# gaebor/w-fsa

Hardware: AMD Instinct MI355X
Metric: forward-backward strings/sec @1/2/4/8 GPU; log-lik rel-err vs MKL ref (higher is better)
Workload: dtype f64

## Files before the change

include/wfsa_dev.h:

```cpp
#ifndef WFSA_DEV_H
#define WFSA_DEV_H

#include <stdint.h>

#ifdef __cplusplus
extern "C" {
#endif

#define WFSA_OK 0
#define WFSA_ERR_ARG (-1)
#define WFSA_ERR_HIP (-2)
#define WFSA_ERR_MODEL (-3)
#define WFSA_ERR_CAPACITY (-4)
#define WFSA_ERR_RCCL (-5)
#define WFSA_ERR_NODEV (-6)

typedef struct wfsa_dev wfsa_dev;

typedef struct {
    int32_t n_states;
    int32_t start;
    int32_t end;
    int32_t n_params;
    const int32_t* em_ptr;
// ... 19 lines not shown
    int64_t stream_bytes;
    int64_t bubble_words;
    int64_t n_bubbles;
    int64_t fb_launches;
    double fb_kernel_ms;
    double last_fb_kernel_ms;
    double last_compiled_ms;
    double last_call_ms;
    int64_t last_live_edges;
    int32_t tier1_strings;
    int32_t waves_per_block;
    double prepare_ms;
    double compiled_kernel_ms;
    int32_t graph;
    int32_t dense;
    int64_t host_steps;
    double host_begin_ms, host_overlap_ms, host_wait_ms, host_post_ms;
    int32_t dense_rows, dense_steps, dense_np;
    int32_t tier2_strings;
    int32_t wave_strings;
    int64_t wave_row_entries;
    int64_t wave_pair_edges;
    int32_t comm_ranks;
    int32_t comm_peer;
    int64_t slot_chunks;
    int32_t max_group_chunks;
    int32_t wave_pull;
    int32_t dense_blas;
    int32_t qn_inkernel_waves;
    int32_t qn_batches;
    int32_t stream_block;
    int32_t stream_w_lds;
    int32_t stream_wide;
    int32_t stream_multi;
    int32_t stream_delta;
    int32_t bubbles_fused;
    int32_t grad_tables;
    int32_t wave_lgrad;
    int64_t ll_dot_launches;
    double best_path_ms;
    double kbest_path_ms;
    double sample_path_ms;
    double posterior_count_ms;
    double byte_marginal_ms;
    int64_t shaped_bubbles;
    int64_t mixed_shape_waves;
    int64_t small_bubbles_a;
    int64_t small_bubbles_b;
    int64_t big_bubbles;
    int32_t max_bubble_nodes;
    int32_t max_bubble_edges;
    double generate_ms;
    double dense_bp_tables_ms, dense_bp_forward_ms, dense_bp_backtrack_ms;
} wfsa_dev_stats;

int wfsa_dev_create(int device, wfsa_dev** out);
void wfsa_dev_destroy(wfsa_dev* ctx);
const char* wfsa_dev_last_error(void);

int wfsa_dev_load_model(wfsa_dev* ctx, const wfsa_model_desc* model);
int wfsa_dev_load_corpus(wfsa_dev* ctx, const uint8_t* sym, const int64_t* off,
                         const double* p, int64_t n_strings);

int wfsa_dev_recognize(wfsa_dev* ctx, uint8_t* recognized, double* path_count,
                       uint8_t* used_param);

int wfsa_dev_sym_factor(wfsa_dev* ctx, int64_t n, const double* a, int64_t inertia[3], double* log_abs_det,
                        int32_t* det_sign);
int wfsa_dev_sym_solve(wfsa_dev* ctx, double* b);
int wfsa_dev_sym_factor_coo(wfsa_dev* ctx, int64_t n, int64_t nnz, const int32_t* i, const int32_t* j,
                            const double* v, double* b, int64_t inertia[3], double* log_abs_det, int32_t* det_sign,
                            int32_t* method);

int wfsa_dev_load_paths(wfsa_dev* ctx, int32_t n_params, int64_t n_paths, const int64_t* prow, const int32_t* pcol,
                        const double* pdata, int64_t n_strings, const int64_t* mrow, const int64_t* mcol,
                        const double* p);

int wfsa_dev_rmin(wfsa_dev* ctx, double* rmin, int64_t* string_index);

int wfsa_dev_best_paths(wfsa_dev* ctx, const double* w_full, double* best_logw, int64_t* n_entries);
int wfsa_dev_best_paths_get(wfsa_dev* ctx, int64_t* prow, int32_t* pidx);

int wfsa_dev_dense_best_paths(wfsa_dev* ctx, const double* w_full, double* best_logw ,
                              int64_t* n_entries );
int wfsa_dev_dense_best_paths_get(wfsa_dev* ctx, int64_t* prow , int32_t* pidx );

#define WFSA_KBEST_MAX 16
int wfsa_dev_kbest_paths(wfsa_dev* ctx, const double* w_full, int32_t k, int64_t* n_paths, int64_t* n_entries);
int wfsa_dev_kbest_paths_get(wfsa_dev* ctx, int64_t* srow , double* logw ,
                             int64_t* prow , int32_t* pidx );

#define WFSA_SAMPLE_MAX 64
int wfsa_dev_sample_paths(wfsa_dev* ctx, const double* w_full, int32_t n, uint64_t seed,
                          double* logq , int64_t* n_paths, int64_t* n_entries );
int wfsa_dev_sample_paths_get(wfsa_dev* ctx, int64_t* srow , double* logw ,
                              int64_t* prow , int32_t* pidx );
int wfsa_dev_sample_uniforms(int device, uint64_t seed, int64_t string, int32_t sample, int32_t n_draws, double* out);

int wfsa_dev_posterior_counts(wfsa_dev* ctx, const double* w_full, double* logq ,
                              double* entropy , int64_t* n_entries );
int wfsa_dev_posterior_counts_get(wfsa_dev* ctx, int64_t* crow , int32_t* cidx ,
                                  double* cval );

int wfsa_dev_byte_marginals(wfsa_dev* ctx, const double* w_full, int32_t decode, double* logq ,
                            double* boundary , double* score ,
                            double* path_logw , int64_t* n_entries, int64_t* n_path_entries);
// ... 57 lines not shown
```

w-fsa_amd/csrc/fb_kernels.hpp:

```cpp
#pragma once

#include <hip/hip_runtime.h>

#include "peer_layout.hpp"

#include <cstddef>
#include <cstdint>
#include <cstdlib>

#ifdef WFSA_EXPERIMENTS
#define WFSA_KDBG(x) (x)
inline int experiment_knob(const char* name) {
    const char* e = std::getenv(name);
    return e ? std::atoi(e) : 0;
}
#else
#define WFSA_KDBG(x) 0
inline int experiment_knob(const char*) { return 0; }
#endif

namespace wfsa {

constexpr int kMaxBubbleNodes = 32;
constexpr int kMaxBubbleEdges = 255;
// ... 520 lines not shown
    const unsigned* halted;
};
struct Publish {
    double* host_out;
    int32_t n;
    const double* add;
    unsigned* seq;
    unsigned* host_flag;
};

__device__ __forceinline__ double strided_sum(const double* __restrict__ p, int n, int t, int nt) {
    double s = 0.0;
    for (int i0 = t; i0 < n; i0 += 8 * nt) {
        double v[8];
#pragma unroll
        for (int b = 0; b < 8; ++b) v[b] = p[min(i0 + b * nt, n - 1)];
#pragma unroll
        for (int b = 0; b < 8; ++b)
            if (i0 + b * nt < n) s += v[b];
    }
    return s;
}

hipError_t configure_kernels(int max_dynamic_lds);
hipError_t launch_trav(TravMode mode, const TravArgs& a, int grid, hipStream_t stream);
hipError_t launch_stream_headers(uint4* stream, const int64_t* g_base, const int32_t* g_len, const double* p_lane,
                                int32_t n_groups, int32_t wide, hipStream_t s);
hipError_t launch_compiled(const CompiledArgs& a, int grid, int block, size_t lds, hipStream_t stream,
                           hipEvent_t ev0 = nullptr, hipEvent_t ev1 = nullptr);
constexpr int kBubbleBlock = 128;
__host__ __device__ inline int64_t small_chunks(int64_t n4, int64_t ns) { return (n4 + 63) / 64 + (ns + 63) / 64; }
__host__ __device__ inline int64_t small_entry(int64_t c, int l, int64_t n4, int64_t ns) {
    const int64_t na = (n4 + 63) / 64;
    if (c < na) {
        const int64_t b = c * 64 + l;
        return b < n4 ? b : -1;
    }
    const int64_t b = n4 + (c - na) * 64 + l;
    return b < n4 + ns ? b : -1;
}
int bubble_waves(int32_t n_small4, int32_t n_small, int32_t n_big);
int fbs_qn_blocks_per_cu(int block, size_t lds);
hipError_t launch_step_dot(const CompiledArgs& a, int grid, int block, size_t lds, hipStream_t stream,
                           hipEvent_t ev0 = nullptr, hipEvent_t ev1 = nullptr);
int step_dot_blocks_per_cu(int block, size_t lds, bool rmin, bool px);
hipError_t launch_bubbles(const BubbleArgs& a, hipStream_t stream);
hipError_t launch_reduce(const ReduceArgs& a, hipStream_t stream);
hipError_t launch_logq_bubbles(double* logq, const double* lz, const int32_t* bpos, const int4* strs, int32_t n,
                               const unsigned* halted, hipStream_t stream);
hipError_t launch_slab_sum(const double* gpart, int32_t n_slabs, int32_t n_params, double* out, hipStream_t stream);
hipError_t launch_publish(const double* out, const Publish& pub, hipStream_t stream);
hipError_t launch_stage(const double* host_w, double* w, double* ewp, int32_t n, hipStream_t stream);
hipError_t launch_qn_step(const QnArgs& a, bool fused, hipStream_t stream);
hipError_t launch_gather(const double* src, const int32_t* idx, int32_t n, double* dst, hipStream_t stream);
hipError_t launch_qn_finish(const QnFinish& f, hipStream_t stream);
hipError_t launch_qn_weights(const double* x, const int32_t* trim, int32_t n_full, double* w_full, double* ewp,
                             hipStream_t stream);
hipError_t launch_copy(const double* src, double* dst, int64_t n, hipStream_t stream);
hipError_t launch_edge_weights(const double* w_full, const int32_t* pptr, const int32_t* pidx, double* lw,
                               double* ew, EdgeRec* erec, int64_t n_edges, double* out, int64_t n_out,
                               hipStream_t stream);
hipError_t launch_node_end(const int32_t* x_ptr, const double* x_w, double* node_end, int32_t n_nodes,
                           hipStream_t stream);

}
```

w-fsa_amd/csrc/qn_kernel.hip:

```cpp
#include "fb_kernels.hpp"
#include "qn_device.hpp"

#include <hip/hip_runtime.h>

#include <algorithm>
#include <cmath>
#include <cstdint>
#include <cstdlib>

#pragma clang fp contract(off)

namespace wfsa {

namespace {

template <bool FUSED, int NT = kQnBlock>
__global__ __launch_bounds__(NT) void qn_step_kernel(QnArgs a) {
    const int t = int(threadIdx.x);
    const int c = int(blockIdx.x);
    extern __shared__ __attribute__((aligned(16))) double qlds[];
    double* sg = qlds;
    double* se = sg + a.seg_cap;
    double* cp = se + a.seg_cap;
    int* sp = reinterpret_cast<int*>(cp + a.chunk_cap);
// ... 126 lines not shown
                if (m >= nm) break;
                const double gi = sg[m], ei = se[m];
                const double aux = ei * lam;
                gerr = fmax(gerr, fabs(gi + aux));
                const double xn = xr[i] - a.eta * ((gi + ei * laux) / aux);
                const int fo = sfo[m];
                a.x[b + m] = xn;
                a.grad[b + m] = gi;
                a.w_full[fo] = xn;
                a.ewp[fo] = exp(xn);
            }
        } else {
            double gs = 0.0, gv = 0.0;
            for (int i = b + t; i < e; i += NT) {
                const double ex = exp(a.x[i]);
                const int fo = a.full_of[i];
                double gi = a.out[1 + fo];
                if (a.fixed) gi += a.fixed[fo];
                a.expx[i] = ex;
                a.grad[i] = gi;
                gs += ex;
                gv += gi;
            }
            gs = block_reduce(gs, 2, red);
            gv = block_reduce(gv, 2, red);
            g = -1.0 + gs;
            laux = (lam * g - gv) / (g + 1.0);
            for (int i = b + t; i < e; i += NT) {
                const double ex = a.expx[i], gi = a.grad[i];
                const double aux = ex * lam;
                gerr = fmax(gerr, fabs(gi + aux));
                const double xn = a.x[i] - a.eta * ((gi + ex * laux) / aux);
                a.x[i] = xn;
                a.w_full[a.full_of[i]] = xn;
                a.ewp[a.full_of[i]] = exp(xn);
            }
        }
        if (t == 0) {
            const double d = lam - laux;
            a.lambda[c] = a.exp_lambda ? lam * exp(-a.eta * (d / lam)) : lam - a.eta * d;
        }
    }
    gerr = (e - b <= 64) ? wave_reduce(gerr, 1) : block_reduce(gerr, 1, red);
    if (t == 0) {
        double4 pv;
        pv.x = have ? g : INFINITY;
        pv.y = have ? g : -INFINITY;
        pv.z = have ? lam : INFINITY;
        pv.w = gerr;
        reinterpret_cast<double4*>(a.partial)[c] = pv;
    }
}

template <bool PX>
__global__ __launch_bounds__(kQnBlock) void qn_finish_kernel(QnFinish f) {
    if (f.halted[0] || f.halted[1]) return;
    __shared__ double red[kMaxBlockWaves];
    qn_finish<PX>(f, red);
}

__global__ void qn_weights_kernel(const double* x, const int32_t* trim, int32_t n_full, double* w_full, double* ewp) {
    const int j = int(blockIdx.x * blockDim.x + threadIdx.x);
    if (j < n_full) {
        const int tj = trim[j];
        w_full[j] = tj >= 0 ? x[tj] : (tj == -1 ? 0.0 : -INFINITY);
        ewp[j] = exp(w_full[j]);
    }
    if (j == n_full) {
        w_full[j] = 0.0;
        ewp[j] = 1.0;
    }
}

}

hipError_t launch_qn_step(const QnArgs& a_in, bool fused, hipStream_t stream) {
    static const int dbg = experiment_knob("WFSA_QN_DBG");
    QnArgs a = a_in;
    a.dbg = dbg;
    if (a.seg_cap <= 0 || a.seg_cap > kQnMaxSeg) a.seg_cap = kQnMaxSeg;
    if (a.chunk_cap <= 0 || a.chunk_cap > kMaxChunks) a.chunk_cap = kMaxChunks;
    const size_t lds = (2 * size_t(a.seg_cap) + size_t(a.chunk_cap)) * sizeof(double) +
                       (3 * size_t(a.seg_cap) + 2) * sizeof(int);
    dim3 grid(unsigned(std::max({a.k, 1, a.rm_on ? a.rm_blocks : 0})));
    if (dbg == 4) {
        grid = dim3(unsigned(std::max((a.k + 3) / 4, 1)));
        a.dbg = 3;
    }
    if (fused) hipLaunchKernelGGL((qn_step_kernel<true>), grid, dim3(kQnBlock), lds, stream, a);
    else hipLaunchKernelGGL((qn_step_kernel<false>), grid, dim3(kQnBlock), lds, stream, a);
    return hipGetLastError();
}

__global__ void copy_kernel(const double* __restrict__ src, double* __restrict__ dst, int64_t n) {
    const int64_t i = int64_t(blockIdx.x) * blockDim.x + threadIdx.x;
    if (i < n) dst[i] = src[i];
}

__global__ void gather_kernel(const double* src, const int32_t* idx, int32_t n, double* dst) {
    const int i = int(blockIdx.x * blockDim.x + threadIdx.x);
    if (i < n) dst[i] = src[idx[i]];
}

hipError_t launch_gather(const double* src, const int32_t* idx, int32_t n, double* dst, hipStream_t stream) {
    if (n <= 0) return hipSuccess;
    hipLaunchKernelGGL(gather_kernel, dim3(unsigned((n + 255) / 256)), dim3(256), 0, stream, src, idx, n, dst);
    return hipGetLastError();
}

hipError_t launch_qn_finish(const QnFinish& f, hipStream_t stream) {
    if (f.px.on) hipLaunchKernelGGL(qn_finish_kernel<true>, dim3(1), dim3(kQnBlock), 0, stream, f);
    else hipLaunchKernelGGL(qn_finish_kernel<false>, dim3(1), dim3(kQnBlock), 0, stream, f);
    return hipGetLastError();
}

hipError_t launch_copy(const double* src, double* dst, int64_t n, hipStream_t stream) {
    if (n <= 0) return hipSuccess;
    hipLaunchKernelGGL(copy_kernel, dim3(unsigned((n + 255) / 256)), dim3(256), 0, stream, src, dst, n);
    return hipGetLastError();
}

hipError_t launch_qn_weights(const double* x, const int32_t* trim, int32_t n_full, double* w_full, double* ewp,
                             hipStream_t stream) {
    const unsigned blocks = unsigned((n_full + 1 + 255) / 256);
    hipLaunchKernelGGL(qn_weights_kernel, dim3(blocks), dim3(256), 0, stream, x, trim, n_full, w_full, ewp);
    return hipGetLastError();
}

}
```

w-fsa_amd/csrc/wfsa_dev.hip:

```cpp
#include "wfsa_dev.h"

#include <hip/hip_runtime.h>

#include <algorithm>
#include <chrono>
#include <cstdarg>
#include <cstdlib>
#include <queue>
#include <cstdio>
#include <cstring>
#include <memory>
#include <limits>
#include <map>
#include <set>
#include <string>
#include <thread>
#include <unordered_map>
#include <vector>

#include "collective.hpp"
#include "dense_path.hpp"
#include "matrix_path.hpp"
#include "sym_solver.hpp"
#include "fb_kernels.hpp"
// ... 267 lines not shown
    bool weights_staged = false;
    bool logq_ready = false;

    bool qn_ready = false;
    int32_t qn_n = 0, qn_k = 0, qn_exp_lambda = 0;
    double qn_plogp = 0.0;
    DevBuf<int32_t> qn_trim, qn_full_of, qn_ccol, qn_cptr;
    int prep_gen = 0;
    DevBuf<double> qn_x, qn_lambda, qn_expx, qn_grad, qn_partial;
    wfsa::QnFinish fin_next{}, fin_for_fbs{};
    DevBuf<double> ll_stash;
    std::vector<int32_t> h_cptr;
    bool fin_pending = false, fin_hostable = false;
    bool fin_next_px = false, fin_for_fbs_px = false;
    wfsa::PeerX cur_px{};
    DevBuf<unsigned> qn_halted;
    std::vector<int32_t> qn_full_of_h, qn_cptr_h;
    bool qn_fused = false;
    int64_t pipe_init_key = -1;
    const double* pipe_init_w = nullptr;
    const double* pipe_init_e = nullptr;
    DevBuf<double> w_full2, ewp2;
    double* w_cur = nullptr;
    double* ewp_cur = nullptr;
    double* qn_ring = nullptr;
    double* qn_ring_dev = nullptr;
    bool use_qw = true;
    int32_t qw_waves = 0;
    double qw_cost = 6.0;
    bool qw_ok = false;
    int32_t qw_nbatch = 0;
    DevBuf<int4> qw_batch;
    DevBuf<int32_t> qw_con_of, qw_mnch, qw_mfirst;
    DevBuf<double> qw_gch;
    int64_t qw_agree_key = -1;
    bool qw_agreed = false;
    std::vector<int64_t> h_mchunk;
    std::vector<int32_t> h_mnch;
    int64_t layout_gen = 0;
    int64_t qw_key = -1;
    std::vector<int4> h_qw_batch;
    DevBuf<unsigned> qw_arrive;
    DevBuf<unsigned> qw_done;
    DevBuf<unsigned> qw_go;
    size_t qw_res_lds = ~size_t(0);
    int qw_res_block = 0, qw_res_per_cu = 0, qw_res_variant = -1;
    uint32_t qw_poll_limit = 0;
    bool qw_poll_fault = false;
    bool qw_last_self = true;
    bool use_ll_dot = true;
    bool use_bubble_shapes = true;
    uint64_t qw_seq = 0;
    wfsa::QnWave qw_next{};
    DevBuf<unsigned long long> fbs_trace;

    std::unique_ptr<wfsa::DensePath> dense;
    int dense_mode = -1;
    bool dense_struct = false;

    bool hf_ready = false;
    int hf_gen = -1;
    std::vector<int32_t> hf_pairs;
    DevBuf<int64_t> hf_slot_base, hf_t_ptr, hf_t_slot;
    DevBuf<double> hf_slot_val, hf_out;
    int64_t hf_n_slots = 0;
    DevBuf<int4> hft_list;
    DevBuf<int32_t> hft_v;
    DevBuf<int64_t> hft_base;
    DevBuf<double> hft_scratch;
    int32_t hft_n = 0;
    int hft_grid = 0;
    int64_t hft_stride = 0;
    int32_t hft_vm = 0;

    int32_t max_dst = 1;
    int64_t n_in_edges = 0;
    DecodeBufs bp, kb;
    DecodeBufs sp;
    DevBuf<double> sp_hist, sp_logq;
    std::vector<int64_t> sp_srow, sp_prow;
    std::vector<double> sp_logw;
    std::vector<int32_t> sp_pidx;
    DecodeBufs pc;
    DevBuf<double> pc_hist, pc_logq, pc_ent, pc_val;
    DevBuf<unsigned long long> pc_gamma, pc_count, pc_cursor;
    DevBuf<int64_t> pc_start;
    DevBuf<int32_t> pc_len, pc_idx;
    std::vector<int64_t> pc_crow;
    std::vector<int32_t> pc_cidx;
    std::vector<double> pc_cval;
    DecodeBufs bm;
    wfsa::MarginalTables bm_tab;
    DevBuf<int32_t> bm_ord, bm_seg, bm_grp;
    DevBuf<int64_t> bm_base;
    bool bm_base_ok = false;
    int64_t bm_words = 0;
    DevBuf<double> bm_hist, bm_logq, bm_bound, bm_score;
    DevBuf<unsigned long long> bm_gamma, bm_mass;
    bool bm_has_path = false;
    std::vector<int64_t> bm_mrow, bm_prow;
    std::vector<int32_t> bm_midx, bm_pidx;
    std::vector<double> bm_mval;
    std::vector<int64_t> bp_prow;
    std::vector<int32_t> bp_pidx;
    bool dbp_valid = false;
    std::vector<int64_t> dbp_prow;
// ... 2262 lines not shown
        if (ctx->comm) {
            if (!ctx->comm->peer_exchange(w.px)) return fail(WFSA_ERR_RCCL, "the peer exchange is not available");
            ctx->cur_px = w.px;
        }
        w.poll_fault = ctx->qw_poll_fault ? 1 : 0;
        if (ctx->qn_rmin) {
            ctx->rm_bpart_cur = ctx->rm_bpart.ptr + size_t(par) * 2 * size_t(ctx->i_grid);
            f.rmin_part = ctx->rm_bpart_cur;
            f.rmin_n_part = ctx->i_grid;
        }
        w.fin = f;
        self_fin = last && ctx->qw_last_self;
        if (self_fin) {
            w.self_finish = 1;
            w.fin.px = w.px;
            w.fin.px_slot = 1;
            w.fin.ll_part = ctx->ll_cur;
            w.fin.n_ll = ctx->i_grid + ((ctx->n_bubbles > 0 && !bubbles_fused(ctx, false)) ? ctx->b_waves : 0) +
                         trav_ll_waves(ctx);
        }
        ++ctx->qw_seq;
    }
    ctx->rm_eval = fuse_rmin;
    const int erc = enqueue_evaluation(ctx, false, ctx->qn_halted.ptr, timed ? slot : -1, !fused && !inkern && trellis,
                                       &n_ll);
    ctx->rm_eval = false;
    ctx->rm_bpart_cur = nullptr;
    if (erc) return erc;
    if (ctx->qw_next.on) return fail(WFSA_ERR_HIP, "the in-kernel QN update was not launched");
    if (fused || inkern) f.n_ll = n_ll;
    if (inkern && self_fin) {
        const int32_t want = ctx->i_grid + ((ctx->n_bubbles > 0 && !bubbles_fused(ctx, false)) ? ctx->b_waves : 0) +
                             trav_ll_waves(ctx);
        if (n_ll != want) return fail(WFSA_ERR_HIP, "self-finish: %d log-likelihood partials, not %d", n_ll, want);
        ctx->fin_pending = false;
        ctx->fin_next.active = 0;
        return WFSA_OK;
    }
    if (ctx->comm && !inkern) COMM_TRY(ctx, ctx->out.ptr, size_t(np) + 1, wfsa::RedOp::SumF64, s);
    if (ctx->qn_rmin && !inkern) {
        constexpr bool fold_rmin = true;
        double* res = ctx->rm_res.ptr + 2 * par;
        if (ctx->mpath || (ctx->dense && !ctx->comm)) {
            if (int rc = enqueue_rmin(ctx, ctx->qn_halted.ptr, res)) return rc;
            f.rmin = res;
        } else if (ctx->comm) {
            if (int rc = enqueue_rmin(ctx, ctx->qn_halted.ptr, res, par, nullptr, true)) return rc;
            if (int rc = combine_rmin(ctx, res, s)) return rc;
            f.rmin = res;
        } else if (int rc = enqueue_rmin(ctx, ctx->qn_halted.ptr, res, par, &f, true, fold_rmin ? &q : nullptr)) {
            return rc;
        }
    }
    if (!inkern) HIP_TRY(wfsa::launch_qn_step(q, fused, s));
    ctx->fin_next = f;
    ctx->fin_next.active = 1;
    ctx->fin_next_px = inkern && ctx->comm;
    ctx->fin_pending = true;
    ctx->fin_hostable = (fused || (trellis && ctx->comm)) && ctx->n_groups > 0 && f.ll_part != nullptr;
    return WFSA_OK;
}

int flush_qn_finish(wfsa_dev* ctx) {
    if (!ctx->fin_pending) return WFSA_OK;
    ctx->fin_pending = false;
    if (ctx->fin_next_px) {
        if (!ctx->comm || !ctx->comm->peer_exchange(ctx->fin_next.px))
            return fail(WFSA_ERR_RCCL, "the peer exchange is not available");
        ctx->fin_next.px_slot = 0;
    }
    HIP_TRY(wfsa::launch_qn_finish(ctx->fin_next, ctx->stream));
    return WFSA_OK;
}

void drop_graph(wfsa_dev* ctx) {
    if (ctx->graph_exec) (void)hipGraphExecDestroy(ctx->graph_exec);
    if (ctx->graph) (void)hipGraphDestroy(ctx->graph);
    if (ctx->graph_exec_nq) (void)hipGraphExecDestroy(ctx->graph_exec_nq);
    if (ctx->graph_nq) (void)hipGraphDestroy(ctx->graph_nq);
    ctx->graph_exec = ctx->graph_exec_nq = nullptr;
    ctx->graph = ctx->graph_nq = nullptr;
    ctx->graph_last = false;
    ctx->graph_failed = false;
}

void invalidate_decodes(wfsa_dev* ctx) {
    ctx->bp.valid = ctx->kb.valid = ctx->sp.valid = ctx->pc.valid = ctx->bm.valid = false;
    ctx->gn_valid = false;
    ctx->dbp_valid = false;
    ctx->bm_base_ok = false;
}

int alloc_param_buffers(wfsa_dev* ctx) {
    HIP_TRY(ctx->w_full.alloc(size_t(ctx->n_params) + 2));
    HIP_TRY(ctx->ewp.alloc(size_t(ctx->n_params) + 2));
    HIP_TRY(ctx->out.alloc(size_t(ctx->n_params) + 2));
    const size_t pinned_need = weights_off(ctx->n_params) + size_t(ctx->n_params) + 2;
    if (ctx->pinned_n < pinned_need) {
        if (ctx->pinned) (void)hipHostFree(ctx->pinned);
        ctx->pinned = nullptr;
        HIP_TRY(hipHostMalloc(reinterpret_cast<void**>(&ctx->pinned), pinned_need * sizeof(double),
                              hipHostMallocMapped | hipHostMallocCoherent));
        HIP_TRY(hipHostGetDevicePointer(reinterpret_cast<void**>(&ctx->pinned_dev), ctx->pinned, 0));
        ctx->pinned_n = pinned_need;
        std::memset(ctx->pinned, 0, pinned_need * sizeof(double));
    }
    return WFSA_OK;
// ... 77 lines not shown
    ctx->prep_level = 0;
    if (!ctx->has_corpus) return WFSA_OK;
    const size_t S = size_t(ctx->n_strings);
    std::vector<int64_t> off(S + 1);
    std::vector<double> p(std::max<size_t>(S, 1));
    HIP_TRY(ctx->off.download(off.data(), S + 1, s));
    HIP_TRY(ctx->p.download(p.data(), S, s));
    HIP_TRY(hipStreamSynchronize(s));
    std::vector<uint8_t> sym(std::max<size_t>(size_t(off[S]), 1));
    HIP_TRY(ctx->sym.download(sym.data(), size_t(off[S]), s));
    HIP_TRY(hipStreamSynchronize(s));
    return dense_load_corpus(ctx, sym.data(), off.data(), p.data());
}

}

extern "C" {

const char* wfsa_dev_last_error(void) { return g_last_error.c_str(); }

int wfsa_dev_create(int device, wfsa_dev** out) {
    if (!out) return fail(WFSA_ERR_ARG, "null output pointer");
    *out = nullptr;
    int n = 0;
    hipError_t e = hipGetDeviceCount(&n);
    if (e != hipSuccess || n == 0)
        return fail(WFSA_ERR_NODEV, "no HIP device available (%s)", e == hipSuccess ? "count 0" : hipGetErrorString(e));
    if (device < 0 || device >= n) return fail(WFSA_ERR_ARG, "device %d out of range (%d devices)", device, n);
    hipDeviceProp_t prop;
    HIP_TRY(hipGetDeviceProperties(&prop, device));
    if (std::strncmp(prop.gcnArchName, "gfx950", 6) != 0)
        return fail(WFSA_ERR_NODEV, "device %d is %s; this build targets gfx950 (MI355X) only", device, prop.gcnArchName);
    HIP_TRY(hipSetDevice(device));
    HIP_TRY(wfsa::configure_kernels(kLdsPerCu));
    std::unique_ptr<wfsa_dev> ctx(new wfsa_dev());
    ctx->device = device;
    ctx->n_cu = prop.multiProcessorCount > 0 ? prop.multiProcessorCount : kNumCu;
    if (const char* e = std::getenv("WFSA_GRAPH")) ctx->use_graph = e[0] == '1';
    if (const char* e = std::getenv("WFSA_TIMING")) ctx->kernel_timing = e[0] != '0';
    if (const char* e = std::getenv("WFSA_DELTA")) ctx->use_delta = e[0] != '0';
    if (const char* e = std::getenv("WFSA_DENSE"); e && e[0]) ctx->dense_mode = e[0] == '0' ? 0 : 1;
    if (const char* e = std::getenv("WFSA_TIER2")) ctx->force_tier2 = e[0] == '1';
    if (const char* e = std::getenv("WFSA_WIDE2")) ctx->use_wide2 = e[0] != '0';
    if (const char* e = std::getenv("WFSA_PULL")) ctx->use_pull = e[0] != '0';
    if (const char* e = std::getenv("WFSA_QN_INKERNEL")) {
        ctx->use_qw = e[0] != '0';
        ctx->qw_force = e[0] == '1';
    }
    if (const char* e = std::getenv("WFSA_FAULT_QN_POLL"); e && e[0] == '1') {
        ctx->qw_poll_fault = true;
        ctx->qw_poll_limit = 256;
    }
    if (const char* e = std::getenv("WFSA_QN_LAST_SELF")) ctx->qw_last_self = e[0] != '0';
    if (const char* e = std::getenv("WFSA_LL_DOT")) ctx->use_ll_dot = e[0] != '0';
    if (const char* e = std::getenv("WFSA_BUBBLE_SHAPES")) ctx->use_bubble_shapes = e[0] != '0';

    HIP_TRY(hipStreamCreateWithFlags(&ctx->stream, hipStreamNonBlocking));
    HIP_TRY(hipEventCreate(&ctx->ev0));
    HIP_TRY(hipEventCreate(&ctx->ev1));
    for (int i = 0; i < kQnDepth; ++i)
        for (hipEvent_t* ev : {&ctx->k0[i], &ctx->kc[i], &ctx->k2[i]}) HIP_TRY(hipEventCreate(ev));
    HIP_TRY(ctx->live.alloc(1));
    HIP_TRY(hipHostMalloc(reinterpret_cast<void**>(&ctx->flag), 64, hipHostMallocMapped | hipHostMallocCoherent));
    HIP_TRY(hipHostGetDevicePointer(reinterpret_cast<void**>(&ctx->flag_dev), ctx->flag, 0));
    *ctx->flag = 0;
    HIP_TRY(ctx->counters.alloc(1));
    HIP_TRY(hipMemsetAsync(ctx->counters.ptr, 0, sizeof(unsigned), ctx->stream));
    HIP_TRY(ctx->qw_arrive.alloc(2));
    HIP_TRY(hipMemsetAsync(ctx->qw_arrive.ptr, 0, 2 * sizeof(unsigned), ctx->stream));
    constexpr size_t n_go = size_t(wfsa::kQnMaxWaves) * wfsa::kQnGoStride;
    HIP_TRY(ctx->qw_go.alloc(n_go));
    HIP_TRY(hipMemsetAsync(ctx->qw_go.ptr, 0, n_go * sizeof(unsigned), ctx->stream));
    HIP_TRY(ctx->qw_done.alloc(2));
    HIP_TRY(hipMemsetAsync(ctx->qw_done.ptr, 0, 2 * sizeof(unsigned), ctx->stream));
    HIP_TRY(hipStreamSynchronize(ctx->stream));
    *out = ctx.release();
    return WFSA_OK;
}

void wfsa_dev_destroy(wfsa_dev* ctx) {
    if (!ctx) return;
    (void)hipSetDevice(ctx->device);
    if (ctx->stream) (void)hipStreamSynchronize(ctx->stream);
    drop_graph(ctx);
    ctx->comm.reset();
    if (ctx->pinned) (void)hipHostFree(ctx->pinned);
    if (ctx->flag) (void)hipHostFree(ctx->flag);
    for (hipEvent_t ev : {ctx->ev0, ctx->ev1})
        if (ev) (void)hipEventDestroy(ev);
    for (DecodeBufs* d : {&ctx->bp, &ctx->kb, &ctx->sp, &ctx->pc, &ctx->bm})
        for (hipEvent_t ev : {d->ev0, d->ev1})
            if (ev) (void)hipEventDestroy(ev);
    for (hipEvent_t ev : ctx->gn_ev)
        if (ev) (void)hipEventDestroy(ev);
    for (hipEvent_t ev : ctx->dbp_ev)
        if (ev) (void)hipEventDestroy(ev);
    for (int i = 0; i < kQnDepth; ++i)
        for (hipEvent_t ev : {ctx->k0[i], ctx->kc[i], ctx->k2[i]})
            if (ev) (void)hipEventDestroy(ev);
    if (ctx->qn_ring) (void)hipHostFree(ctx->qn_ring);
    if (ctx->qst) (void)hipHostFree(ctx->qst);
    if (ctx->stream) (void)hipStreamDestroy(ctx->stream);
    delete ctx;
}

int wfsa_dev_load_model(wfsa_dev* ctx, const wfsa_model_desc* model) {
// ... 566 lines not shown
        for (int32_t c = 0; c < k; ++c) sz.push_back(ctx->h_seg_ptr[size_t(cptr[size_t(c) + 1])] - ctx->h_seg_ptr[size_t(cptr[size_t(c)])]);
        std::sort(sz.begin(), sz.end());
        if (!sz.empty())
            std::fprintf(stderr, "[wfsa] slots per constraint: total %lld, max %lld, p99 %lld, p50 %lld\n",
                         (long long)ctx->h_seg_ptr.back(), (long long)sz.back(), (long long)sz[sz.size() * 99 / 100],
                         (long long)sz[sz.size() / 2]);
    }
    hipStream_t s = ctx->stream;
    mark(6);
    if (!ctx->qn_flags_clear) HIP_TRY(hipMemsetAsync(ctx->qn_halted.ptr, 0, 3 * sizeof(unsigned), s));
    ctx->qn_flags_clear = false;
    ctx->fin_pending = false;
    ctx->fin_for_fbs.active = 0;
    const int64_t ft_key = ctx->prep_gen * 1000003 + ctx->qn_setup_gen;
    if (ctx->qn_fused && !ctx->dense && !ctx->mpath && ctx->n_groups > 0 && ctx->qn_n > 0) {
        if (!ctx->fixed_t_on || ctx->fixed_t_key != ft_key) {
            HIP_TRY(ctx->fixed_t.alloc(size_t(ctx->qn_n)));
            HIP_TRY(wfsa::launch_gather(ctx->fixed_grad.ptr, ctx->qn_full_of.ptr, ctx->qn_n, ctx->fixed_t.ptr, s));
            ctx->fixed_t_on = true;
            ctx->fixed_t_key = ft_key;
        }
    } else {
        ctx->fixed_t_on = false;
    }
    mark(1);
    if (ctx->use_qw && ctx->qw_waves > 0)
        if (int rc = build_qw_batches(ctx)) return rc;
    mark(2);
    bool inkern = qw_usable(ctx);
    mark(3);
    if (ctx->comm) {
        const int64_t key = ((ctx->prep_gen * 1000003 + ctx->qn_setup_gen) * 1000003 + ctx->layout_gen) * 2 +
                            (ctx->qn_rmin ? 1 : 0);
        if (ctx->qw_agree_key != key) {
            double bad = inkern ? 0.0 : 1.0;
            HIP_TRY(ctx->qw_gch.alloc(std::max<size_t>(ctx->qw_gch.n, 1)));
            HIP_TRY(hipMemcpyAsync(ctx->qw_gch.ptr, &bad, sizeof bad, hipMemcpyHostToDevice, s));
            COMM_TRY(ctx, ctx->qw_gch.ptr, 1, wfsa::RedOp::SumF64, s);
            HIP_TRY(hipMemcpyAsync(&bad, ctx->qw_gch.ptr, sizeof bad, hipMemcpyDeviceToHost, s));
            HIP_TRY(hipStreamSynchronize(s));
            COMM_CHECK(ctx);
            ctx->qw_agree_key = key;
            ctx->qw_agreed = bad == 0.0;
        }
        inkern = ctx->qw_agreed;
    }
    if (!inkern && ctx->use_qw && std::getenv("WFSA_VERBOSE"))
        std::fprintf(stderr, "[wfsa] QN update as its own kernel: cover %d (%.1f rows per wave) batches %d waves %d "
                     "fused %d comm %d rmin %d delta %d fallback %d bubbles fused %d fixed_t %d k %d\n", int(ctx->qw_cover),
                     ctx->qw_mean_rows, int(ctx->qw_ok), ctx->qw_waves, int(ctx->qn_fused),
                     int(ctx->comm != nullptr), int(ctx->qn_rmin), int(ctx->delta_on),
                     ctx->n_fall[0] + ctx->n_fall[1] + ctx->n_fall[2],
                     int(ctx->n_bubbles == 0 || bubbles_fused(ctx, false)), int(ctx->fixed_t_on), ctx->qn_k);
    ctx->stats.qn_inkernel_waves = inkern ? ctx->qw_waves : 0;
    ctx->stats.qn_batches = inkern ? ctx->qw_nbatch : 0;
    if (inkern) {
        HIP_TRY(ctx->w_full2.alloc(size_t(ctx->n_params) + 2));
        HIP_TRY(ctx->ewp2.alloc(size_t(ctx->n_params) + 2));
        if (ctx->pipe_init_key != ft_key || ctx->pipe_init_w != ctx->w_full2.ptr || ctx->pipe_init_e != ctx->ewp2.ptr) {
            HIP_TRY(hipMemcpyAsync(ctx->w_full2.ptr, ctx->w_full.ptr, (size_t(ctx->n_params) + 2) * sizeof(double),
                                   hipMemcpyDeviceToDevice, s));
            HIP_TRY(hipMemcpyAsync(ctx->ewp2.ptr, ctx->ewp.ptr, (size_t(ctx->n_params) + 2) * sizeof(double),
                                   hipMemcpyDeviceToDevice, s));
            ctx->pipe_init_key = ft_key;
            ctx->pipe_init_w = ctx->w_full2.ptr;
            ctx->pipe_init_e = ctx->ewp2.ptr;
        }
    }
    mark(4);
    auto timed_step = [&](int32_t e) {
        const int32_t k = ctx->timing_stride;
        return e % k == k - 1 || (max_steps < k && e == max_steps - 1);
    };
    const unsigned base = ctx->seq;
    int32_t enq = 0, done = 0, st = 0;
    bool stop = false;
    double c_ms_sum = 0.0, fb_ms_sum = 0.0;
    int64_t timed = 0;
    if (trace) tr_pro = clk::now();
    while (done < max_steps) {
        while (!stop && enq < max_steps && enq - done < (ctx->dense ? 2 : kQnDepth)) {
            const bool tm = timed_step(enq);
            if (int rc = enqueue_qn_step(ctx, eta, tol, enq, tm, inkern, enq + 1 == max_steps))
                return rc;
            ++enq;
            ++ctx->seq;
            if (trace && enq == 1) tr_enq1 = clk::now();
        }
        if (stop || enq == max_steps)
            if (int rc = flush_qn_finish(ctx)) return rc;
        if (done >= enq) break;
        if (int rc = wait_published(ctx, base + unsigned(done) + 1u)) return rc;
        if (trace) (done == 0 ? tr_first : tr_last) = clk::now();
        const int slot = done % kQnDepth;
        const double* row = ctx->qn_ring + size_t(slot) * wfsa::kQnRow;
        if (int rc = wait_row(ctx, row, base + unsigned(done) + 1u)) return rc;
        const unsigned rs = unsigned(uint64_t(row[7]) & 15u);
        if (ctx->kernel_timing && timed_step(done)) {
            float c = 0.f, f = 0.f;
            const hipEvent_t end = ctx->k2_kc[slot] ? ctx->kc[slot] : ctx->k2[slot];
            hipError_t q;
            while ((q = hipEventQuery(end)) == hipErrorNotReady) __builtin_ia32_pause();
            if (q == hipSuccess &&
                hipEventElapsedTime(&c, ctx->k0[slot], ctx->kc[slot]) == hipSuccess &&
                hipEventElapsedTime(&f, ctx->k0[slot], end) == hipSuccess) {
                c_ms_sum += c;
// ... 1480 lines not shown
```

w-fsa_amd/wfsa_amd/_lib.py:

```python
import ctypes as C
import os

HERE = os.path.dirname(os.path.abspath(__file__))
LIB_PATH = os.environ.get("WFSA_LIB") or os.path.join(HERE, "libwfsa_amd.so")

WFSA_OK = 0
WFSA_ERR_ARG = -1
WFSA_ERR_HIP = -2
WFSA_ERR_MODEL = -3
WFSA_ERR_CAPACITY = -4
WFSA_ERR_RCCL = -5
WFSA_ERR_NODEV = -6
COMM_ID_BYTES = 128

vp = C.c_void_p
i32, i64, u8, dbl = C.c_int32, C.c_int64, C.c_uint8, C.c_double
P = C.POINTER


class ModelDesc(C.Structure):
    _fields_ = [
        ("n_states", i32), ("start", i32), ("end", i32), ("n_params", i32),
        ("em_ptr", P(i32)), ("em_off", P(i64)), ("em_len", P(i32)), ("em_param", P(i32)),
        ("em_bytes", P(u8)), ("tr_ptr", P(i32)), ("tr_dst", P(i32)), ("tr_param", P(i32)),
    ]


class DevStats(C.Structure):
    _fields_ = [
        ("n_strings", i64), ("total_symbols", i64), ("max_len", i32), ("n_nodes", i32),
        ("n_edges", i64), ("n_end_edges", i64), ("compiled_strings", i64), ("fallback_strings", i64),
        ("stream_words", i64), ("stream_bytes", i64), ("bubble_words", i64), ("n_bubbles", i64), ("fb_launches", i64), ("fb_kernel_ms", dbl),
        ("last_fb_kernel_ms", dbl), ("last_compiled_ms", dbl), ("last_call_ms", dbl),
        ("last_live_edges", i64), ("tier1_strings", i32), ("waves_per_block", i32), ("prepare_ms", dbl),
        ("compiled_kernel_ms", dbl), ("graph", i32), ("dense", i32),
        ("host_steps", i64), ("host_begin_ms", dbl), ("host_overlap_ms", dbl), ("host_wait_ms", dbl),
        ("host_post_ms", dbl),
        ("dense_rows", i32), ("dense_steps", i32), ("dense_np", i32), ("tier2_strings", i32),
        ("wave_strings", i32), ("wave_row_entries", i64), ("wave_pair_edges", i64),
        ("comm_ranks", i32), ("comm_peer", i32),
        ("slot_chunks", i64), ("max_group_chunks", i32), ("wave_pull", i32),
        ("dense_blas", i32), ("qn_inkernel_waves", i32), ("qn_batches", i32),
        ("stream_block", i32), ("stream_w_lds", i32), ("stream_wide", i32), ("stream_multi", i32),
        ("stream_delta", i32), ("bubbles_fused", i32), ("grad_tables", i32), ("wave_lgrad", i32),
        ("ll_dot_launches", i64), ("best_path_ms", dbl), ("kbest_path_ms", dbl),
        ("sample_path_ms", dbl), ("posterior_count_ms", dbl), ("byte_marginal_ms", dbl),
        ("shaped_bubbles", i64), ("mixed_shape_waves", i64), ("small_bubbles_a", i64), ("small_bubbles_b", i64),
        ("big_bubbles", i64), ("max_bubble_nodes", i32), ("max_bubble_edges", i32),
        ("generate_ms", dbl),
        ("dense_bp_tables_ms", dbl), ("dense_bp_forward_ms", dbl), ("dense_bp_backtrack_ms", dbl),
    ]


HOST_ALLREDUCE_FN = C.CFUNCTYPE(C.c_int, vp, vp, i64, i32)


class LearnerInfo(C.Structure):
    _fields_ = [
        ("n_strings", i64), ("n_local_strings", i64), ("n_paths", i64),
        ("n_full", i32), ("n_params", i32), ("n_constraints", i32), ("unique_paths", i32),
        ("aux_params", i64),
        ("common_support", dbl), ("plogp", dbl), ("model_volume", dbl), ("aux_hessian", dbl),
        ("kl", dbl), ("loglik", dbl), ("shard_begin", i64), ("shard_end", i64),
    ]


_SIGS = {
    "wfsa_dev_create": (C.c_int, [C.c_int, P(vp)]),
    "wfsa_dev_destroy": (None, [vp]),
    "wfsa_dev_last_error": (C.c_char_p, []),
    "wfsa_dev_load_model": (C.c_int, [vp, P(ModelDesc)]),
    "wfsa_dev_load_corpus": (C.c_int, [vp, vp, vp, vp, i64]),
    "wfsa_dev_recognize": (C.c_int, [vp, vp, vp, vp]),
    "wfsa_dev_string_tiers": (C.c_int, [vp, vp]),
    "wfsa_dev_rmin": (C.c_int, [vp, vp, vp]),
    "wfsa_dev_best_paths": (C.c_int, [vp, vp, vp, P(i64)]),
    "wfsa_dev_best_paths_get": (C.c_int, [vp, vp, vp]),
    "wfsa_dev_dense_best_paths": (C.c_int, [vp, vp, vp, P(i64)]),
    "wfsa_dev_dense_best_paths_get": (C.c_int, [vp, vp, vp]),
    "wfsa_dev_kbest_paths": (C.c_int, [vp, vp, C.c_int32, P(i64), P(i64)]),
    "wfsa_dev_kbest_paths_get": (C.c_int, [vp, vp, vp, vp, vp]),
    "wfsa_dev_sample_paths": (C.c_int, [vp, vp, C.c_int32, C.c_uint64, vp, P(i64), P(i64)]),
    "wfsa_dev_sample_paths_get": (C.c_int, [vp, vp, vp, vp, vp]),
    "wfsa_dev_generate": (C.c_int, [vp, vp, i64, C.c_int32, C.c_uint64, P(i64), P(i64), vp]),
    "wfsa_dev_generate_get": (C.c_int, [vp, vp, vp, vp, vp, vp, vp, vp]),
    "wfsa_dev_posterior_counts": (C.c_int, [vp, vp, vp, vp, P(i64)]),
    "wfsa_dev_posterior_counts_get": (C.c_int, [vp, vp, vp, vp]),
    "wfsa_dev_byte_marginals": (C.c_int, [vp, vp, C.c_int32, vp, vp, vp, vp, P(i64), P(i64)]),
    "wfsa_dev_byte_marginals_get": (C.c_int, [vp, vp, vp, vp]),
    "wfsa_dev_byte_marginals_path_get": (C.c_int, [vp, vp, vp]),
    "wfsa_dev_sample_uniforms": (C.c_int, [C.c_int, C.c_uint64, i64, C.c_int32, C.c_int32, vp]),
    "wfsa_dev_sym_factor": (C.c_int, [vp, C.c_int64, vp, vp, vp, vp]),
    "wfsa_dev_sym_solve": (C.c_int, [vp, vp]),
    "wfsa_dev_sym_factor_coo": (C.c_int, [vp, C.c_int64, C.c_int64, vp, vp, vp, vp, vp, vp, vp, vp]),
    "wfsa_dev_load_paths": (C.c_int, [vp, C.c_int32, C.c_int64, vp, vp, vp, C.c_int64, vp, vp, vp]),
    "wfsa_learner_load_matrices": (C.c_int, [vp, C.c_char_p]),
    "wfsa_learner_set_info_rmin": (C.c_int, [vp, C.c_int]),
    "wfsa_learner_save_matrices": (C.c_int, [vp, C.c_char_p]),
    "wfsa_dev_objective_grad": (C.c_int, [vp, vp, P(dbl), vp, vp]),
    "wfsa_dev_objective_grad_begin": (C.c_int, [vp, vp, C.c_int]),
    "wfsa_dev_weights_staging": (vp, [vp]),
    "wfsa_dev_objective_grad_end": (C.c_int, [vp, P(dbl), vp, vp]),
    "wfsa_dev_qn_setup": (C.c_int, [vp, vp]),
# ... 108 lines not shown
```

Baseline: 56.93 billion.

## Add wave-per-constraint fused QN step kernel with DPP chunk reductions

Adds a new quasi-Newton step kernel that maps one constraint group to one 64-lane wavefront. Contributions are summed per chunk with DPP cross-lane adds and staged in LDS, then each member thread accumulates its own chunk range, and the group sums and lambda update run inside the wave using only wave-level barriers. It is selected by default for fused, non-in-kernel steps whenever every group has few enough members and chunks, and otherwise falls back to the existing step kernel. This aims to cut the per-step reduction and synchronisation cost, but adds a second code path whose summation order differs from the old kernel and can change floating-point rounding.

```diff
diff --git a/include/wfsa_dev.h b/include/wfsa_dev.h
--- a/include/wfsa_dev.h
+++ b/include/wfsa_dev.h
@@ -95,6 +95,7 @@
     int32_t max_bubble_edges;
     double generate_ms;
     double dense_bp_tables_ms, dense_bp_forward_ms, dense_bp_backtrack_ms;
+    int64_t qn_wave_launches;
 } wfsa_dev_stats;
 
 int wfsa_dev_create(int device, wfsa_dev** out);
diff --git a/w-fsa_amd/csrc/fb_kernels.hpp b/w-fsa_amd/csrc/fb_kernels.hpp
--- a/w-fsa_amd/csrc/fb_kernels.hpp
+++ b/w-fsa_amd/csrc/fb_kernels.hpp
@@ -596,6 +596,8 @@
 hipError_t launch_publish(const double* out, const Publish& pub, hipStream_t stream);
 hipError_t launch_stage(const double* host_w, double* w, double* ewp, int32_t n, hipStream_t stream);
 hipError_t launch_qn_step(const QnArgs& a, bool fused, hipStream_t stream);
+constexpr int kQnWaveMaxChunks = 64 * kQnWaveChunkRounds;
+hipError_t launch_qn_wave(const QnArgs& a, hipStream_t stream);
 hipError_t launch_gather(const double* src, const int32_t* idx, int32_t n, double* dst, hipStream_t stream);
 hipError_t launch_qn_finish(const QnFinish& f, hipStream_t stream);
 hipError_t launch_qn_weights(const double* x, const int32_t* trim, int32_t n_full, double* w_full, double* ewp,
diff --git a/w-fsa_amd/csrc/qn_kernel.hip b/w-fsa_amd/csrc/qn_kernel.hip
--- a/w-fsa_amd/csrc/qn_kernel.hip
+++ b/w-fsa_amd/csrc/qn_kernel.hip
@@ -202,6 +202,124 @@
     }
 }
 
+constexpr int kQnWaveLds = kQnWaveMaxChunks + 2 * kQnWaveMembers;
+__device__ __forceinline__ void qn_wave_sync() {
+    __builtin_amdgcn_fence(__ATOMIC_SEQ_CST, "wavefront");
+    __builtin_amdgcn_wave_barrier();
+    __builtin_amdgcn_fence(__ATOMIC_SEQ_CST, "wavefront");
+}
+template <int CTRL>
+__device__ __forceinline__ double qn_dpp(double v) {
+    int lo = __double2loint(v), hi = __double2hiint(v);
+    lo = __builtin_amdgcn_update_dpp(lo, lo, CTRL, 0xf, 0xf, false);
+    hi = __builtin_amdgcn_update_dpp(hi, hi, CTRL, 0xf, 0xf, false);
+    return __hiloint2double(hi, lo);
+}
+__global__ __launch_bounds__(kQnBlock) void qn_wave_kernel(QnArgs a) {
+    if (WFSA_KDBG(a.dbg) == 3) return;
+    __shared__ __attribute__((aligned(16))) double wlds[kQnBlock / 64][kQnWaveLds];
+    const int lane = int(threadIdx.x) & 63;
+    const int wv = __builtin_amdgcn_readfirstlane(int(threadIdx.x) >> 6);
+    const int c = int(blockIdx.x) * (kQnBlock / 64) + wv;
+    const unsigned h0 = a.halted[0], h1 = a.halted[1];
+    if (c >= a.k) return;
+    const int b = a.cptr[c], e = a.cptr[c + 1];
+    const double lam = a.lambda[c];
+    const int64_t gb = a.grp_base[c];
+    const int gnch = WFSA_KDBG(a.dbg) == 5 ? 0 : a.grp_nch[c];
+    if (h0 || h1) {
+        if (c == 0 && lane == 0) {
+            a.halted[0] = 1u;
+            qn_publish_row(a.fin, nullptr, kQnSkipped);
+        }
+        return;
+    }
+    double* cp = wlds[wv];
+    double* se = cp + kQnWaveMaxChunks;
+    double* sg = se + kQnWaveMembers;
+    const int nm = min(e - b, kQnWaveMembers);
+    const int gn = min(gnch, kQnWaveMaxChunks);
+    const bool valid = lane < nm;
+    const int i = b + (valid ? lane : 0);
+    const double x = a.x[i], ft = a.fixed_t[i];
+    const int fo = a.full_of[i];
+    const int q0a = a.chunk_ptr[i], q1a = a.chunk_ptr[i + 1];
+    const double gout = a.use_out ? a.out[1 + fo] : 0.0;
+    if (WFSA_KDBG(a.dbg) == 1) {
+        if (x + ft + gout + double(q0a + q1a) == 0.12345) a.partial[0] = lam + double(gb + gn);
+        return;
+    }
+    const double2* v2 = reinterpret_cast<const double2*>(a.contrib + gb);
+    const int sub = lane & 7;
+    for (int cb0 = 0; cb0 < gn; cb0 += 64) {
+        double2 y[8];
+#pragma unroll
+        for (int r = 0; r < 8; ++r) {
+            const int q = cb0 + 8 * r + (lane >> 3);
+            y[r] = q < gn ? v2[size_t(q) * 8 + sub] : make_double2(0.0, 0.0);
+        }
+#pragma unroll
+        for (int r = 0; r < 8; ++r) {
+            double sr = y[r].x + y[r].y;
+            sr += qn_dpp<0xB1>(sr);
+            sr += qn_dpp<0x4E>(sr);
+            sr += qn_dpp<0x141>(sr);
+            const int q = cb0 + 8 * r + (lane >> 3);
+            if (sub == 0 && q < gn) cp[q] = sr;
+        }
+    }
+    qn_wave_sync();
+    const int c0 = __builtin_amdgcn_readfirstlane(q0a);
+    double sm = 0.0;
+    if (valid) {
+        int q = q0a - c0;
+        const int q1 = min(q1a - c0, gn);
+        for (; q + 8 <= q1; q += 8) {
+            double t[8];
+#pragma unroll
+            for (int k = 0; k < 8; ++k) t[k] = cp[q + k];
+#pragma unroll
+            for (int k = 0; k < 8; ++k) sm += t[k];
+        }
+        for (; q < q1; ++q) sm += cp[q];
+    }
+    double gi = gout;
+    gi += ft;
+    gi = gi + sm;
+    const double ei = exp(x);
+    if (valid) {
+        se[lane] = ei;
+        sg[lane] = gi;
+    }
+    qn_wave_sync();
+    double gg = -1.0;
+    for (int m = 0; m < nm; ++m) gg += se[m];
+    double r = lam * gg;
+    for (int m = 0; m < nm; ++m) r -= sg[m];
+    const double laux = r / (gg + 1.0);
+    double gerr = 0.0;
+    if (valid) {
+        const double aux = ei * lam;
+        gerr = fmax(gerr, fabs(gi + aux));
+        const double xn = x - a.eta * ((gi + ei * laux) / aux);
+        a.x[i] = xn;
+        a.grad[i] = gi;
+        a.w_full[fo] = xn;
+        a.ewp[fo] = exp(xn);
+    }
+    gerr = wave_reduce(gerr, 1);
+    if (lane == 0) {
+        const double d = lam - laux;
+        a.lambda[c] = a.exp_lambda ? lam * exp(-a.eta * (d / lam)) : lam - a.eta * d;
+        double4 pv;
+        pv.x = gg;
+        pv.y = gg;
+        pv.z = lam;
+        pv.w = gerr;
+        reinterpret_cast<double4*>(a.partial)[c] = pv;
+    }
+}
+
 template <bool PX>
 __global__ __launch_bounds__(kQnBlock) void qn_finish_kernel(QnFinish f) {
     if (f.halted[0] || f.halted[1]) return;
@@ -242,6 +360,16 @@
     return hipGetLastError();
 }
 
+hipError_t launch_qn_wave(const QnArgs& a_in, hipStream_t stream) {
+    static const int dbg = experiment_knob("WFSA_QN_DBG");
+    if (a_in.k <= 0 || !a_in.contrib || !a_in.fixed_t || a_in.rm_on || a_in.ll_stash) return hipErrorInvalidValue;
+    QnArgs a = a_in;
+    a.dbg = dbg;
+    constexpr int WPB = kQnBlock / 64;
+    hipLaunchKernelGGL(qn_wave_kernel, dim3(unsigned((a.k + WPB - 1) / WPB)), dim3(kQnBlock), 0, stream, a);
+    return hipGetLastError();
+}
+
 __global__ void copy_kernel(const double* __restrict__ src, double* __restrict__ dst, int64_t n) {
     const int64_t i = int64_t(blockIdx.x) * blockDim.x + threadIdx.x;
     if (i < n) dst[i] = src[i];
diff --git a/w-fsa_amd/csrc/wfsa_dev.hip b/w-fsa_amd/csrc/wfsa_dev.hip
--- a/w-fsa_amd/csrc/wfsa_dev.hip
+++ b/w-fsa_amd/csrc/wfsa_dev.hip
@@ -343,6 +343,8 @@
     bool use_bubble_shapes = true;
     uint64_t qw_seq = 0;
     wfsa::QnWave qw_next{};
+    bool use_qn_wave = true;
+    bool qnw_ok = false;
     DevBuf<unsigned long long> fbs_trace;
 
     std::unique_ptr<wfsa::DensePath> dense;
@@ -2711,7 +2713,14 @@
             return rc;
         }
     }
-    if (!inkern) HIP_TRY(wfsa::launch_qn_step(q, fused, s));
+    const bool wave = !inkern && fused && ctx->use_qn_wave && ctx->qnw_ok && ctx->fixed_t_on && !q.rm_on &&
+                      q.contrib != nullptr && !q.ll_stash;
+    if (wave) {
+        HIP_TRY(wfsa::launch_qn_wave(q, s));
+        ++ctx->stats.qn_wave_launches;
+    } else if (!inkern) {
+        HIP_TRY(wfsa::launch_qn_step(q, fused, s));
+    }
     ctx->fin_next = f;
     ctx->fin_next.active = 1;
     ctx->fin_next_px = inkern && ctx->comm;
@@ -2895,6 +2904,7 @@
         ctx->qw_poll_limit = 256;
     }
     if (const char* e = std::getenv("WFSA_QN_LAST_SELF")) ctx->qw_last_self = e[0] != '0';
+    if (const char* e = std::getenv("WFSA_QN_WAVE")) ctx->use_qn_wave = e[0] != '0';
     if (const char* e = std::getenv("WFSA_LL_DOT")) ctx->use_ll_dot = e[0] != '0';
     if (const char* e = std::getenv("WFSA_BUBBLE_SHAPES")) ctx->use_bubble_shapes = e[0] != '0';
 
@@ -3567,6 +3577,12 @@
                      int(ctx->comm != nullptr), int(ctx->qn_rmin), int(ctx->delta_on),
                      ctx->n_fall[0] + ctx->n_fall[1] + ctx->n_fall[2],
                      int(ctx->n_bubbles == 0 || bubbles_fused(ctx, false)), int(ctx->fixed_t_on), ctx->qn_k);
+    ctx->qnw_ok = ctx->qn_fused && ctx->qn_k > 0 && int64_t(ctx->h_cptr.size()) == int64_t(ctx->qn_k) + 1 &&
+                  ctx->lead_grp_nch <= wfsa::kQnWaveMaxChunks;
+    for (int32_t c = 0; ctx->qnw_ok && c < ctx->qn_k; ++c) {
+        const int32_t nm = ctx->h_cptr[size_t(c) + 1] - ctx->h_cptr[size_t(c)];
+        ctx->qnw_ok = nm >= 1 && nm <= wfsa::kQnWaveMembers;
+    }
     ctx->stats.qn_inkernel_waves = inkern ? ctx->qw_waves : 0;
     ctx->stats.qn_batches = inkern ? ctx->qw_nbatch : 0;
     if (inkern) {
diff --git a/w-fsa_amd/wfsa_amd/_lib.py b/w-fsa_amd/wfsa_amd/_lib.py
--- a/w-fsa_amd/wfsa_amd/_lib.py
+++ b/w-fsa_amd/wfsa_amd/_lib.py
@@ -49,6 +49,7 @@
         ("big_bubbles", i64), ("max_bubble_nodes", i32), ("max_bubble_edges", i32),
         ("generate_ms", dbl),
         ("dense_bp_tables_ms", dbl), ("dense_bp_forward_ms", dbl), ("dense_bp_backtrack_ms", dbl),
+        ("qn_wave_launches", i64),
     ]
 
 
```

New measurement: 63.56 billion (median of 6 runs). 1.12x the previous value.
